# leotimus/binary-recommendation

Hardware: AMD Instinct MI355X
Metric: (user,item) pairs/sec at batch 65536 dim 64 (higher is better)
Workload: dtype f32; 1 GPU; NeuMF-A full training step (trainers/NFC_plain.py graph: 4 embeddings, 128->100->50->10->1, BCE, Keras-Adam adam_dense), embed_dim=64, 1000000 users x 100000 items per GPU, batch 65536 per GPU, uniform ids; global_batch=65536, parallelism=single GPU, steps_per_graph_launch=4, optimizer=adam_dense (deferred replay)

## Files before the change

### binary-recommendation_amd/csrc/dense.h

```cpp
#pragma once
#include "common.h"
#include "philox.h"
#include <stdlib.h>

namespace br {

typedef __bf16 bf16x8 __attribute__((ext_vector_type(8)));
typedef float f32x4_t __attribute__((ext_vector_type(4)));
__device__ __forceinline__ void split3(float x0, float x1, uint32_t& h, uint32_t& m, uint32_t& l) {
  typedef __bf16 bf2 __attribute__((ext_vector_type(2)));
  typedef float f2 __attribute__((ext_vector_type(2)));
  const f2 x = {x0, x1};
  h = __builtin_bit_cast(uint32_t, (bf2){(__bf16)x.x, (__bf16)x.y});
  const f2 hf = {__builtin_bit_cast(float, h << 16), __builtin_bit_cast(float, h & 0xffff0000u)};
  const f2 r = x - hf;
  m = __builtin_bit_cast(uint32_t, (bf2){(__bf16)r.x, (__bf16)r.y});
  const f2 mf = {__builtin_bit_cast(float, m << 16), __builtin_bit_cast(float, m & 0xffff0000u)};
  const f2 t = r - mf;
  l = __builtin_bit_cast(uint32_t, (bf2){(__bf16)t.x, (__bf16)t.y});
}
__device__ __forceinline__ bf16x8 frag8(const uint32_t (&p)[4]) {
  typedef uint32_t u4 __attribute__((ext_vector_type(4)));
  const u4 v = {p[0], p[1], p[2], p[3]};
  return __builtin_bit_cast(bf16x8, v);
}
__device__ __forceinline__ bf16x8 frag8(const float4& q) {
  typedef float f4 __attribute__((ext_vector_type(4)));
  const f4 v = {q.x, q.y, q.z, q.w};
  return __builtin_bit_cast(bf16x8, v);
}
__device__ __forceinline__ f32x4_t mfma_bf16(bf16x8 a, bf16x8 b, f32x4_t c) {
#if defined(__HIP_DEVICE_COMPILE__)
  return __builtin_amdgcn_mfma_f32_16x16x32_bf16(a, b, c, 0, 0, 0);
#else
  return c;
#endif
}
static inline bool mlp_bf16x6() {
  static const bool on = [] { const char* e = getenv("BR_MLP_MATH"); return !(e && e[0] == 'f'); }();
  return on;
}

struct BwdArgs {
  const float* gy; int64_t ldgy;
  const float* y; int64_t ldy;
  const float* x; int64_t ldx;
  const float* W;
  int64_t batch;
  int K, N, act;
  const float* o_mean; const float* o_rstd; const float* o_gamma; const double* o_sums; float inv_batch;
  const float* scale; const float* shift;
  const uint32_t* keep; int kw; float inv_keep;
  const float* i_mean; const float* i_rstd; double* in_sums;
  float* gx; int64_t ldgx;
  float* slabs; int64_t slab_elems; int64_t db_off;
  float* zero = nullptr; int64_t zero_n = 0;
};

int make_keep_args(KeepArgs& a, float drop_p, uint64_t seed, uint32_t step, uint32_t step_add, int64_t row0, int64_t batch, int n_sites,
                   const uint32_t* sites, const int* widths, uint32_t* const* out);
int dropout_keep_bits_ahead(float drop_p, uint64_t seed, uint32_t step, uint32_t step_add, int64_t row0, int64_t batch, int n_sites,
                            const uint32_t* sites, const int* widths, uint32_t* const* out, brStream stream);

struct AdamPairCall {
  float *table_a, *m_a, *v_a; int64_t rows_a; const void* sorted_ids_a; const int32_t* sorted_pos_a; const float* grads_a; int64_t ldg_a;
  const float* grads_hi_a; int64_t ldg_hi_a; uint8_t* mark_a; int32_t* last_a;
  float *table_b, *m_b, *v_b; int64_t rows_b; const void* sorted_ids_b; const int32_t* sorted_pos_b; const float* grads_b; int64_t ldg_b;
  const float* grads_hi_b; int64_t ldg_hi_b; uint8_t* mark_b; int32_t* last_b;
  int dim, id_type; int64_t n; int split; const float* hi_scale; const void* step_state; double alpha_t, beta1, beta2, eps;
  float *seg_ws_a, *seg_ws_b;
  const float *th_lo_a = nullptr, *th_hi_a = nullptr, *th_lo_b = nullptr, *th_hi_b = nullptr; int64_t ld_th = 0;
  const StepAdvance* adv = nullptr;
};
struct FinalArgs;
int adam_rows_pair_keep(const AdamPairCall& c, const KeepArgs* keep, brStream stream, const FinalArgs* fin = nullptr, bool* fin_done = nullptr);

struct LookupArgs;
struct IndexPairArgs {
  void* sorted_ids_a; int32_t* sorted_pos_a; void* ws_a; int64_t ws_a_bytes;
  void* sorted_ids_b; int32_t* sorted_pos_b; void* ws_b; int64_t ws_b_bytes;
};
bool lookup_with_index_supported(int dim, int64_t n, int64_t upper_a, int64_t upper_b, int64_t ld_stash, const void* x0, const void* stash_a, const void* stash_b);
struct GroupIndexArgs { int n = 0; const void* users[BR_GROUP_MAX - 1]; const void* items[BR_GROUP_MAX - 1]; IndexPairArgs ix[BR_GROUP_MAX - 1]; };
int lookup_with_index(const LookupArgs& la, int dim, int id_type, const IndexPairArgs& ix, brStream stream, const StepAdvance* adv = nullptr,
                      const GroupIndexArgs* later = nullptr);
int lookup_index_chunks(int64_t n);
int lookup_wave_launch(const LookupArgs& la, int dim, int id_type, brStream stream);

int dense_backward_fused(const BwdArgs& a, hipStream_t s);
int dense_bwd_fused_grid(int64_t batch);
size_t dense_bwd_fused_lds(int NT, int KT);

struct TailMArgs {
  const float* a2; int64_t lda2;
  const float *W3, *b3, *w4, *b4, *dot, *labels;
  const float *scale2, *shift2, *mean2, *rstd2;
  const double* stats2; double batch_total; const float *gamma2, *beta2; float bn_eps, bn_momentum;
  float *moving_mean, *moving_var, *out_scale, *out_shift, *out_mean, *out_rstd;
  const uint32_t* keep; int kw; float inv_keep;
  int64_t batch;
  int n2, n3, act, mf_first, loss;
  float inv_batch;
  float *a3, *logit, *prob, *ddot, *gh2;
  int64_t ldgh2;
  double *msums, *bn_sums;
  float* slabs; int n_slabs;
};
int tail_mfma_grid(int64_t batch);
void launch_tail_mfma(const TailMArgs& a, int grid, hipStream_t s);

}
```

### binary-recommendation_amd/csrc/stamps.h

```cpp
#pragma once
#include "common.h"

namespace br {

#ifdef BR_STAMPS
constexpr int kStampSlots = 12;
__device__ unsigned long long* g_stamp_buf = nullptr;
#define BR_STAMP_DECL unsigned long long stamps_[kStampSlots] = {0, 0, 0, 0, 0, 0, 0, 0, 0, 0, 0, 0}
#define BR_STAMP(i)                                                                             \
  do {                                                                                          \
    __builtin_amdgcn_sched_barrier(0);                                                          \
    unsigned long long t_;                                                                      \
    asm volatile("s_memtime %0\n\ts_waitcnt lgkmcnt(0)" : "=s"(t_)::"memory");                  \
    if (stamps_[i] == 0) stamps_[i] = t_;                                                       \
    __builtin_amdgcn_sched_barrier(0);                                                          \
  } while (0)
#define BR_STAMP_RT(i)                                                                          \
  do {                                                                                          \
    unsigned long long t_;                                                                      \
    asm volatile("s_memrealtime %0\n\ts_waitcnt lgkmcnt(0)" : "=s"(t_)::"memory");              \
    stamps_[i] = t_;                                                                            \
  } while (0)
#define BR_STAMP_FLUSH(widx)                                                                    \
  do {                                                                                          \
    if ((threadIdx.x & 63) == 0 && g_stamp_buf)                                                 \
      for (int i_ = 0; i_ < kStampSlots; ++i_) g_stamp_buf[(size_t)(widx) * kStampSlots + i_] = stamps_[i_]; \
  } while (0)
#else
#define BR_STAMP_DECL
#define BR_STAMP(i)
#define BR_STAMP_RT(i)
#define BR_STAMP_FLUSH(widx)
#endif

}
```

### binary-recommendation_amd/csrc/tail.hip

```cpp
#include "common.h"
#include "dense.h"

namespace br {

constexpr int kTailRows = 128;
constexpr int kTailLpr = 4;
constexpr int kTailRep = BR_STAT_REPLICAS;

struct TailArgs {
  const float* a2; int64_t lda2;
  const float *W3, *b3, *w4, *b4, *dot, *labels;
  const float *scale2, *shift2, *mean2, *rstd2;
  const uint8_t* keep; int64_t keep_ld; float inv_keep;
  int64_t batch;
  int n2, n3, act, mf_first, loss;
  float inv_batch;
  float *a3, *logit, *prob, *ddot, *gh2;
  int64_t ldgh2;
  double *msums, *bn_sums;
  float* slabs;
};

template <int N3P, int ROWS>
__global__ __launch_bounds__(ROWS * kTailLpr) void neumf_tail_kernel(TailArgs a) {
  constexpr int kTailThreads = ROWS * kTailLpr, kTailWaves = kTailThreads / 64, kPasses = kTailRows / ROWS;
  extern __shared__ __attribute__((aligned(16))) float smem[];
  const int n2 = a.n2, n3 = a.n3, ld = n2 | 1;
  float* A = smem;
  float* X = A + ROWS * ld;
  float* Ws = X + ROWS * ld;
  float* DZ = Ws + n2 * N3P;
  float* cst = DZ + ROWS * (N3P + 1);
  float* hw = cst + 4 * n2;
  float* A3s = hw + 2 * N3P;
  __shared__ float redf[kTailWaves][N3P + 2];
  __shared__ double redd[kTailWaves][BR_METRIC_SUMS];
  __shared__ double colred[2][128];
  const int t = threadIdx.x, lane = t & 63, wave = t >> 6;
  const int r = t >> 2, q = t & 3;
  const int moff = a.mf_first ? 1 : 0;
  const float wdot = a.w4[a.mf_first ? 0 : n3], bias4 = a.b4[0];
  const int64_t base0 = (int64_t)blockIdx.x * kTailRows;
#pragma unroll 1
  for (int pass = 0; pass < kPasses; ++pass) {
  const int64_t base = base0 + (int64_t)pass * ROWS;
  const int64_t left = a.batch - base;
  const int nrow = (int)(left < ROWS ? (left > 0 ? left : 0) : ROWS);
  const bool live = r < nrow;
  const int64_t gr = base + r;
  const float d = live ? a.dot[gr] : 0.f, yv = live ? a.labels[gr] : 0.f;

  {
    constexpr int RPW = ROWS / kTailWaves;
    float v[RPW][2];
#pragma unroll
    for (int i = 0; i < RPW; ++i) {
      const int rr = wave + kTailWaves * i;
      const float* src = a.a2 + (rr < nrow ? base + rr : base0) * a.lda2;
#pragma unroll
      for (int h = 0; h < 2; ++h) {
        const int k = lane + 64 * h;
        const float x = src[k < n2 ? k : 0];
        v[i][h] = (rr < nrow && k < n2) ? x : 0.f;
      }
    }
#pragma unroll
    for (int i = 0; i < RPW; ++i) {
      const int rr = wave + kTailWaves * i;
#pragma unroll
      for (int h = 0; h < 2; ++h) {
        const int k = lane + 64 * h;
        if (k < n2) A[rr * ld + k] = v[i][h];
      }
    }
  }
  if (pass == 0) {
    for (int e = t; e < n2 * N3P; e += kTailThreads) { const int k = e / N3P, n = e - k * N3P; Ws[e] = n < n3 ? a.W3[k * n3 + n] : 0.f; }
    for (int k = t; k < n2; k += kTailThreads) {
      cst[k] = a.scale2[k]; cst[n2 + k] = a.shift2[k]; cst[2 * n2 + k] = a.mean2[k]; cst[3 * n2 + k] = a.rstd2[k];
    }
    for (int n = t; n < N3P; n += kTailThreads) { hw[n] = n < n3 ? a.b3[n] : 0.f; hw[N3P + n] = n < n3 ? a.w4[moff + n] : 0.f; }
  }
  for (int k = t; k < 256; k += kTailThreads) (&colred[0][0])[k] = 0.0;
  __syncthreads();

  const float ik = a.inv_keep;
  float z[N3P];
#pragma unroll
  for (int n = 0; n < N3P; ++n) z[n] = q == 0 ? hw[n] : 0.f;
  uint32_t bits[4];
#pragma unroll
  for (int i = 0; i < 4; ++i) {
    const int k0 = 8 * (q + 4 * i);
    bits[i] = 0u;
    if (k0 < n2) {
      bits[i] = live ? (a.keep ? (uint32_t)a.keep[gr * a.keep_ld + (k0 >> 3)] : 0xFFu) : 0u;
      const int kend = (n2 - k0) < 8 ? (n2 - k0) : 8;
      for (int j = 0; j < kend; ++j) {
        const int k = k0 + j;
        const float h = A[r * ld + k] * cst[k] + cst[n2 + k];
        const float x = ((bits[i] >> j) & 1u) ? h * ik : 0.f;
        X[r * ld + k] = x;
#pragma unroll
        for (int n4 = 0; n4 < N3P; n4 += 4) {
          const float4 w = *reinterpret_cast<const float4*>(Ws + k * N3P + n4);
          z[n4] += x * w.x; z[n4 + 1] += x * w.y; z[n4 + 2] += x * w.z; z[n4 + 3] += x * w.w;
        }
      }
    }
  }
#pragma unroll
  for (int n = 0; n < N3P; ++n) { z[n] += __shfl_xor(z[n], 1, 64); z[n] += __shfl_xor(z[n], 2, 64); }
  float lz = bias4 + d * wdot;
#pragma unroll
  for (int n = 0; n < N3P; ++n) {
    z[n] = n < n3 ? act_apply(z[n], a.act) : 0.f;
    lz += z[n] * hw[N3P + n];
  }
  const float p = sigmoidf_acc(lz);
  float dzl = 0.f;
  double s_loss = 0.0, s_se = 0.0, s_ae = 0.0, s_ok = 0.0, s_bce = 0.0, s_tp = 0.0, s_fp = 0.0, s_fn = 0.0;
  const bool own = live && q == 0;
  if (live) {
    float l;
    const float bce = fmaxf(lz, 0.f) - lz * yv + log1pf(expf(-fabsf(lz)));
    if (a.loss == BR_LOSS_BCE) {
      l = bce;
      dzl = (p - yv) * a.inv_batch;
    } else {
      l = (p - yv) * (p - yv);
      dzl = 2.f * (p - yv) * p * (1.f - p) * a.inv_batch;
    }
    if (own) {
      s_loss = (double)l; s_se = (double)((p - yv) * (p - yv)); s_ae = (double)fabsf(p - yv);
      const bool pp = p > 0.5f, yp = yv > 0.5f;
      s_ok = (pp == yp) ? 1.0 : 0.0;
      s_bce = (double)bce; s_tp = (pp && yp) ? 1.0 : 0.0; s_fp = (pp && !yp) ? 1.0 : 0.0; s_fn = (!pp && yp) ? 1.0 : 0.0;
      a.logit[gr] = lz;
      a.prob[gr] = p;
      a.ddot[gr] = dzl * wdot;
    }
  }
  if (q == 0) {
#pragma unroll
    for (int n = 0; n < N3P; ++n) A3s[r * (N3P + 1) + n] = z[n];
  }
  float dz[N3P];
#pragma unroll
  for (int n = 0; n < N3P; ++n) {
    dz[n] = (live && n < n3) ? dzl * hw[N3P + n] * act_grad_from_out(z[n], a.act) : 0.f;
    if (q == 0) DZ[r * (N3P + 1) + n] = dz[n];
  }
  const float dzo = own ? dzl : 0.f;
#pragma unroll
  for (int n = 0; n < N3P; ++n) {
    const float v = group_sum<64>(dzo * z[n]);
    if (lane == 0) redf[wave][n] = v;
  }
  {
    const float v0 = group_sum<64>(dzo * d), v1 = group_sum<64>(dzo);
    if (lane == 0) { redf[wave][N3P] = v0; redf[wave][N3P + 1] = v1; }
    s_loss = wave_sum_d(s_loss); s_se = wave_sum_d(s_se); s_ae = wave_sum_d(s_ae); s_ok = wave_sum_d(s_ok);
    s_bce = wave_sum_d(s_bce); s_tp = wave_sum_d(s_tp); s_fp = wave_sum_d(s_fp); s_fn = wave_sum_d(s_fn);
    if (lane == 0) {
      redd[wave][0] = s_loss; redd[wave][1] = s_se; redd[wave][2] = s_ae; redd[wave][3] = s_ok;
      redd[wave][4] = s_bce; redd[wave][5] = s_tp; redd[wave][6] = s_fp; redd[wave][7] = s_fn;
    }
  }
  __syncthreads();

  float* slab = a.slabs + (int64_t)blockIdx.x * ((int64_t)n2 * n3 + 2 * n3 + 2);
  for (int o = t; o < n2 * n3; o += kTailThreads) {
    const int k = o / n3, n = o - k * n3;
    float acc = 0.f;
    for (int rr = 0; rr < ROWS; ++rr) acc += X[rr * ld + k] * DZ[rr * (N3P + 1) + n];
    slab[o] = pass ? slab[o] + acc : acc;
  }
  if (a.a3)
    for (int e = t; e < nrow * n3; e += kTailThreads) { const int rr = e / n3; a.a3[base * n3 + e] = A3s[rr * (N3P + 1) + (e - rr * n3)]; }
  auto put = [&](int i, float v) { slab[i] = pass ? slab[i] + v : v; };
  auto wsum = [&](int i) { float v = 0.f; for (int w = 0; w < kTailWaves; ++w) v += redf[w][i]; return v; };
  if (t < n3) {
    float acc = 0.f;
    for (int rr = 0; rr < ROWS; ++rr) acc += DZ[rr * (N3P + 1) + t];
    put(n2 * n3 + t, acc);
    put(n2 * n3 + n3 + moff + t, wsum(t));
  }
  if (t == 64) put(n2 * n3 + n3 + (a.mf_first ? 0 : n3), wsum(N3P));
  if (t == 65) put(n2 * n3 + 2 * n3 + 1, wsum(N3P + 1));
  if (t >= 96 && t < 96 + BR_METRIC_SUMS && a.msums) {
    double v = 0.0;
    for (int w = 0; w < kTailWaves; ++w) v += redd[w][t - 96];
    atomicAdd(a.msums + (size_t)(blockIdx.x & (BR_SUM_SLOTS - 1)) * BR_METRIC_SUMS + (t - 96), v);
  }
  __syncthreads();

#pragma unroll
  for (int i = 0; i < 4; ++i) {
    const int k0 = 8 * (q + 4 * i);
    if (k0 < n2) {
      const int kend = (n2 - k0) < 8 ? (n2 - k0) : 8;
      for (int j = 0; j < kend; ++j) {
        const int k = k0 + j;
        float acc = 0.f;
#pragma unroll
        for (int n4 = 0; n4 < N3P; n4 += 4) {
          const float4 w = *reinterpret_cast<const float4*>(Ws + k * N3P + n4);
          acc += dz[n4] * w.x + dz[n4 + 1] * w.y + dz[n4 + 2] * w.z + dz[n4 + 3] * w.w;
        }
        const float dh = ((bits[i] >> j) & 1u) ? acc * ik : 0.f;
        const float xhat = (A[r * ld + k] - cst[2 * n2 + k]) * cst[3 * n2 + k];
        A[r * ld + k] = dh;
        X[r * ld + k] = dh * xhat;
      }
    }
  }
  __syncthreads();
  if (a.bn_sums) {
    for (int idx = t; idx < 4 * n2; idx += kTailThreads) {
      const int part = idx / n2, k = idx - part * n2;
      float s1 = 0.f, s2 = 0.f;
      for (int rr = part * (ROWS / 4); rr < (part + 1) * (ROWS / 4); ++rr) { s1 += A[rr * ld + k]; s2 += X[rr * ld + k]; }
      atomicAdd(&colred[0][k], (double)s1);
      atomicAdd(&colred[1][k], (double)s2);
    }
  }
  for (int rr = wave; rr < nrow; rr += kTailWaves) {
    float* dst = a.gh2 + (base + rr) * a.ldgh2;
    for (int k = lane; k < n2; k += 64) dst[k] = A[rr * ld + k];
  }
  if (a.bn_sums) {
    __syncthreads();
    double* rep = a.bn_sums + (size_t)(blockIdx.x % kTailRep) * 2 * n2;
    for (int k = t; k < n2; k += kTailThreads) {
      atomicAdd(rep + k, colred[0][k]);
      atomicAdd(rep + n2 + k, colred[1][k]);
    }
  }
  if (kPasses > 1) __syncthreads();
  }
}

static size_t tail_lds_bytes(int n2, int n3p, int rows) {
  const int ld = n2 | 1;
  return sizeof(float) * ((size_t)2 * rows * ld + (size_t)n2 * n3p + (size_t)2 * rows * (n3p + 1) + 4 * (size_t)n2 + 2 * (size_t)n3p);
}
static size_t tail_static_lds_bytes(int n3p, int rows) {
  const int waves = rows * kTailLpr / 64;
  return sizeof(float) * waves * (n3p + 2) + sizeof(double) * (waves * BR_METRIC_SUMS + 2 * 128);
}
constexpr size_t kTailDynLdsMax = 150 * 1024;
constexpr size_t kTailCuLds = 160 * 1024;
static bool tail_fits(int n2, int n3p, int rows) {
  const size_t dyn = tail_lds_bytes(n2, n3p, rows);
  return dyn <= kTailDynLdsMax && dyn + tail_static_lds_bytes(n3p, rows) <= kTailCuLds;
}
static int tail_tile_rows(int n2, int n3p) { return tail_fits(n2, n3p, kTailRows) ? kTailRows : kTailRows / 2; }

}

using namespace br;

extern "C" int brNeumfTailSlabs(int64_t batch) { return (int)ceil_div(batch > 0 ? batch : 1, kTailRows); }

extern "C" int64_t brNeumfTailSlabElems(int n2, int n3) { return (int64_t)n2 * n3 + 2 * n3 + 2; }

extern "C" int brNeumfTailFused(const float* a2, int64_t lda2, const float* W3, const float* b3, const float* w4, const float* b4,
                                const float* dot, const float* labels, const float* scale2, const float* shift2, const float* mean2,
                                const float* rstd2, const brBnFold* bn2, float drop_p, const uint32_t* keep,
                                int64_t batch, int n2, int n3, int act, int mf_first, int loss, float inv_batch, float* a3,
                                float* logit, float* prob, double* sums, float* ddot, float* gh2, int64_t ldgh2, double* bn_sums,
                                float* slabs, int n_slabs, brStream stream) {
  BR_CHECK_ARG(a2 && W3 && b3 && w4 && b4 && dot && labels && logit && prob && ddot && gh2 && slabs, "brNeumfTailFused: null pointer");
  BR_CHECK_ARG(bn2 ? (!scale2 && !shift2 && !mean2 && !rstd2 && bn2->stats && bn2->gamma && bn2->beta && bn2->scale && bn2->shift && bn2->mean && bn2->rstd &&
                      bn2->batch_total > 0 && (bn2->moving_mean == nullptr) == (bn2->moving_var == nullptr))
                   : (scale2 && shift2 && mean2 && rstd2),
               "brNeumfTailFused: BatchNorm 2 either as scale2/shift2/mean2/rstd2 or as bn2 (stats, gamma, beta and the four outputs)");
  BR_CHECK_ARG(batch >= 0 && n2 >= 1 && n2 <= 128 && n3 >= 1 && n3 <= 32 && lda2 >= n2 && ldgh2 >= n2, "brNeumfTailFused: bad sizes");
  BR_CHECK_ARG(drop_p >= 0.f && drop_p < 1.f, "brNeumfTailFused: drop_p out of [0,1)");
  BR_CHECK_ARG((drop_p > 0.f) == (keep != nullptr), "brNeumfTailFused: keep bits (brDropoutKeepBits) are required exactly when drop_p > 0");
  BR_CHECK_ARG(loss == BR_LOSS_BCE || loss == BR_LOSS_MSE, "brNeumfTailFused: bad loss");
  const int n3p = (n3 + 3) & ~3, tile_rows = tail_tile_rows(n2, n3p);
  if (!tail_fits(n2, n3p, tile_rows)) {
    set_error("brNeumfTailFused: n2 = %d with n3 = %d needs %zu B of dynamic LDS (+ %zu B static) for %d-row tiles, above the %zu B a workgroup may "
              "request; the largest supported combination is n2 = 128 with n3 = 32",
              n2, n3, tail_lds_bytes(n2, n3p, tile_rows), tail_static_lds_bytes(n3p, tile_rows), tile_rows, kTailDynLdsMax);
    return BR_ERR_UNSUPPORTED;
  }
  if (batch == 0) return BR_OK;
  BR_CHECK_ARG(n_slabs == brNeumfTailSlabs(batch), "brNeumfTailFused: n_slabs must be brNeumfTailSlabs(batch)");
  hipStream_t s = (hipStream_t)stream;
  const auto al16 = [](const void* p) { return (reinterpret_cast<uintptr_t>(p) & 15) == 0; };
  if (n2 <= 64 && n3 <= 16 && lda2 % 4 == 0 && ldgh2 % 4 == 0 && al16(a2) && al16(gh2)) {
    TailMArgs m{};
    m.a2 = a2; m.lda2 = lda2; m.W3 = W3; m.b3 = b3; m.w4 = w4; m.b4 = b4; m.dot = dot; m.labels = labels;
    m.scale2 = scale2; m.shift2 = shift2; m.mean2 = mean2; m.rstd2 = rstd2;
    if (bn2) {
      m.stats2 = bn2->stats; m.batch_total = bn2->batch_total; m.gamma2 = bn2->gamma; m.beta2 = bn2->beta; m.bn_eps = bn2->eps; m.bn_momentum = bn2->momentum;
      m.moving_mean = bn2->moving_mean; m.moving_var = bn2->moving_var; m.out_scale = bn2->scale; m.out_shift = bn2->shift; m.out_mean = bn2->mean; m.out_rstd = bn2->rstd;
    }
    m.keep = keep; m.kw = (n2 + 31) / 32; m.inv_keep = drop_p > 0.f ? 1.0f / (1.0f - drop_p) : 1.0f;
    m.batch = batch; m.n2 = n2; m.n3 = n3; m.act = act; m.mf_first = mf_first; m.loss = loss; m.inv_batch = inv_batch;
    m.a3 = a3; m.logit = logit; m.prob = prob; m.ddot = ddot; m.gh2 = gh2; m.ldgh2 = ldgh2; m.msums = sums; m.bn_sums = bn_sums; m.slabs = slabs;
    int grid = tail_mfma_grid(batch);
    if (grid > n_slabs) grid = n_slabs;
    m.n_slabs = n_slabs;
    launch_tail_mfma(m, grid, s);
    BR_CHECK_LAUNCH("brNeumfTailFused(mfma)");
    return BR_OK;
  }
  if (bn2) {
    int rc = brBnFinalize(bn2->stats, bn2->batch_total, bn2->gamma, bn2->beta, bn2->eps, bn2->momentum, bn2->moving_mean, bn2->moving_var, bn2->scale,
                          bn2->shift, bn2->mean, bn2->rstd, n2, stream);
    if (rc != BR_OK) return rc;
    scale2 = bn2->scale; shift2 = bn2->shift; mean2 = bn2->mean; rstd2 = bn2->rstd;
  }
  TailArgs a;
  a.a2 = a2; a.lda2 = lda2; a.W3 = W3; a.b3 = b3; a.w4 = w4; a.b4 = b4; a.dot = dot; a.labels = labels;
  a.scale2 = scale2; a.shift2 = shift2; a.mean2 = mean2; a.rstd2 = rstd2;
  a.keep = reinterpret_cast<const uint8_t*>(keep); a.keep_ld = 4 * (int64_t)((n2 + 31) / 32); a.inv_keep = drop_p > 0.f ? 1.0f / (1.0f - drop_p) : 1.0f;
  a.batch = batch; a.n2 = n2; a.n3 = n3; a.act = act; a.mf_first = mf_first; a.loss = loss; a.inv_batch = inv_batch;
  a.a3 = a3; a.logit = logit; a.prob = prob; a.ddot = ddot; a.gh2 = gh2; a.ldgh2 = ldgh2; a.msums = sums; a.bn_sums = bn_sums;
  a.slabs = slabs;
  const size_t lds = tail_lds_bytes(n2, n3p, tile_rows);
  const unsigned grid = (unsigned)n_slabs;
#define BR_TAIL_LAUNCH(NP, ROWS)                                                                                          \
  {                                                                                                                       \
    static bool attr = false;                                                                                             \
    if (!attr) {                                                                                                          \
      const hipError_t e = hipFuncSetAttribute((const void*)neumf_tail_kernel<NP, ROWS>, hipFuncAttributeMaxDynamicSharedMemorySize, (int)kTailDynLdsMax); \
      if (e != hipSuccess) { set_error("brNeumfTailFused: cannot raise the dynamic LDS limit to %zu B: %s", kTailDynLdsMax, hipGetErrorString(e)); return BR_ERR_HIP; } \
      attr = true;                                                                                                        \
    }                                                                                                                     \
    neumf_tail_kernel<NP, ROWS><<<grid, ROWS * kTailLpr, lds, s>>>(a);                                                     \
  }
#define BR_TAIL(NP) case NP: BR_TAIL_LAUNCH(NP, kTailRows) break;
#define BR_TAIL2(NP) case NP: if (tile_rows == kTailRows) BR_TAIL_LAUNCH(NP, kTailRows) else BR_TAIL_LAUNCH(NP, kTailRows / 2) break;
  switch (n3p) {
    BR_TAIL(4) BR_TAIL(8) BR_TAIL2(12) BR_TAIL2(16) BR_TAIL2(20) BR_TAIL2(24) BR_TAIL2(28) BR_TAIL2(32)
    default: set_error("brNeumfTailFused: unsupported n3"); return BR_ERR_UNSUPPORTED;
  }
#undef BR_TAIL
#undef BR_TAIL2
#undef BR_TAIL_LAUNCH
  BR_CHECK_LAUNCH("brNeumfTailFused");
  return BR_OK;
}
```

### binary-recommendation_amd/csrc/tail_mfma.hip

```cpp
#include "dense.h"

namespace br {

using f32x4 = __attribute__((ext_vector_type(4))) float;

constexpr int kTmThreads = 512;
constexpr int kTmWaves = kTmThreads / 64;
constexpr int kTmRep = BR_STAT_REPLICAS;
constexpr int kTmPatchLd = 20;
constexpr int kTmKT = 4;

__device__ __forceinline__ f32x4 mfma16t(float a, float b, f32x4 c) {
  return __builtin_amdgcn_mfma_f32_16x16x4f32(a, b, c, 0, 0, 0);
}
__device__ __forceinline__ float keep_bit_t(float x, uint32_t w, uint32_t pos) {
  return __int_as_float(__float_as_int(x) & __builtin_amdgcn_sbfe((int)w, pos, 1u));
}

struct TailTile {
  float4 av[kTmKT];
  uint32_t ka[2];
  float xr[4][kTmKT], dv[4], yv[4];
  uint32_t kc[4][2];
  int vm[4];
};
__device__ __forceinline__ void tail_load_tile(TailTile& t, const TailMArgs& a, int64_t tile, int c16, int g) {
  const int64_t batch = a.batch, rbase = tile << 4;
  const int n2 = a.n2;
  const int64_t arow = rbase + c16 < batch ? rbase + c16 : batch - 1;
  const float* pa = a.a2 + arow * a.lda2 + 4 * g;
#pragma unroll
  for (int j = 0; j < kTmKT; ++j) t.av[j] = *reinterpret_cast<const float4*>(16 * j + 4 * g < n2 ? pa + 16 * j : pa - 4 * g);
  t.ka[0] = t.ka[1] = 0xFFFFFFFFu;
  if (a.keep) { t.ka[0] = a.keep[arow * a.kw]; t.ka[1] = a.keep[arow * a.kw + (a.kw > 1 ? 1 : 0)]; }
#pragma unroll
  for (int r = 0; r < 4; ++r) {
    const int64_t row = rbase + 4 * g + r;
    t.vm[r] = row < batch ? -1 : 0;
    const int64_t rc = row < batch ? row : batch - 1;
    const float* px = a.a2 + rc * a.lda2;
#pragma unroll
    for (int kt = 0; kt < kTmKT; ++kt) { const int k = kt * 16 + c16; t.xr[r][kt] = px[k < n2 ? k : 0]; }
    t.kc[r][0] = a.keep ? a.keep[rc * a.kw] : 0xFFFFFFFFu;
    t.kc[r][1] = a.keep ? a.keep[rc * a.kw + (a.kw > 1 ? 1 : 0)] : 0xFFFFFFFFu;
    t.dv[r] = a.dot[rc];
    t.yv[r] = a.labels[rc];
  }
}

__global__ __launch_bounds__(kTmThreads, 2) void neumf_tail_mfma_kernel(const TailMArgs a) {
  __shared__ __attribute__((aligned(16))) float Wf[4 * 4 * 16 * 4];
  __shared__ __attribute__((aligned(16))) float Wb[64 * 16];
  __shared__ float cst[4][64];
  __shared__ __attribute__((aligned(16))) float hv[2][16];
  __shared__ __attribute__((aligned(16))) float patches[kTmWaves][16 * kTmPatchLd];
  __shared__ float wsum[kTmWaves][64 * 16];
  __shared__ float wcol[kTmWaves][2][16 + 2];
  __shared__ double wbn[2][64];
  __shared__ double wmet[kTmWaves][BR_METRIC_SUMS];
  const int lane = threadIdx.x & 63, wave = threadIdx.x >> 6;
  const int c16 = lane & 15, g = lane >> 4;
  const int n2 = a.n2, n3 = a.n3;
  const int64_t batch = a.batch;
  const int moff = a.mf_first ? 1 : 0;
  const int sigmask = a.act == BR_ACT_SIGMOID ? -1 : 0, relumask = a.act == BR_ACT_RELU ? -1 : 0;
  const float floor_ = a.act == BR_ACT_RELU ? 0.f : -__builtin_inff();

  const int64_t n_tiles = (batch + 15) >> 4;
  const int64_t tile0 = (int64_t)blockIdx.x * kTmWaves + wave;
  TailTile tt;
  if (tile0 < n_tiles) tail_load_tile(tt, a, tile0, c16, g);
  for (int t = threadIdx.x; t < 64; t += kTmThreads) {
    float sc = 0.f, sh = 0.f, mu = 0.f, rs = 0.f;
    if (t < n2) {
      if (a.stats2) {
        double s1 = 0.0, s2 = 0.0;
        for (int r = 0; r < kTmRep; ++r) { s1 += a.stats2[(size_t)r * 2 * n2 + t]; s2 += a.stats2[(size_t)r * 2 * n2 + n2 + t]; }
        const double m = s1 / a.batch_total;
        double var = s2 / a.batch_total - m * m;
        if (var < 0.0) var = 0.0;
        mu = (float)m;
        const float varf = (float)var;
        rs = 1.0f / sqrtf(varf + a.bn_eps);
        sc = a.gamma2[t] * rs;
        sh = a.beta2[t] - mu * sc;
        if (blockIdx.x == 0) {
          a.out_scale[t] = sc; a.out_shift[t] = sh; a.out_mean[t] = mu; a.out_rstd[t] = rs;
          if (a.moving_mean) {
            a.moving_mean[t] = a.moving_mean[t] * a.bn_momentum + mu * (1.0f - a.bn_momentum);
            a.moving_var[t] = a.moving_var[t] * a.bn_momentum + varf * (1.0f - a.bn_momentum);
          }
        }
      } else { sc = a.scale2[t]; sh = a.shift2[t]; mu = a.mean2[t]; rs = a.rstd2[t]; }
    }
    cst[0][t] = sc; cst[1][t] = sh; cst[2][t] = mu; cst[3][t] = rs;
    wbn[0][t] = 0.0; wbn[1][t] = 0.0;
  }
  for (int t = threadIdx.x; t < 16; t += kTmThreads) {
    hv[0][t] = t < n3 ? a.b3[t] : 0.f;
    hv[1][t] = t < n3 ? a.w4[moff + t] : 0.f;
  }
  for (int t = threadIdx.x; t < 64 * 16; t += kTmThreads) {
    const int k = t >> 4, n = t & 15;
    const float w = (k < n2 && n < n3) ? a.W3[k * n3 + n] : 0.f;
    Wb[t] = w;
    Wf[(((k >> 4) * 4 + ((k >> 2) & 3)) * 16 + n) * 4 + (k & 3)] = w;
  }
  __syncthreads();

  const float wdot = a.w4[a.mf_first ? 0 : n3], bias4 = a.b4[0];
  float* patch = patches[wave];
  f32x4 dW[kTmKT];
#pragma unroll
  for (int kt = 0; kt < kTmKT; ++kt) dW[kt] = (f32x4){0.f, 0.f, 0.f, 0.f};
  float db3 = 0.f, dw4 = 0.f, dw4dot = 0.f, db4 = 0.f;
  float isum[kTmKT], isq[kTmKT];
#pragma unroll
  for (int kt = 0; kt < kTmKT; ++kt) { isum[kt] = 0.f; isq[kt] = 0.f; }
  double s_loss = 0.0, s_se = 0.0, s_ae = 0.0, s_ok = 0.0, s_bce = 0.0, s_tp = 0.0, s_fp = 0.0, s_fn = 0.0;
  const float4 w4q = *reinterpret_cast<const float4*>(&hv[1][4 * g]);
  const float b3c = hv[0][c16], w4c = hv[1][c16];
  const float ik = a.inv_keep;

  for (int64_t tile = tile0; tile < n_tiles; tile += (int64_t)gridDim.x * kTmWaves) {
    const int64_t rbase = tile << 4;
    if (tile != tile0) tail_load_tile(tt, a, tile, c16, g);
    float4 (&av)[kTmKT] = tt.av;
    uint32_t (&ka)[2] = tt.ka;
    float (&xr)[4][kTmKT] = tt.xr;
    float (&dv)[4] = tt.dv;
    float (&yv)[4] = tt.yv;
    uint32_t (&kc)[4][2] = tt.kc;
    int (&vm)[4] = tt.vm;
    f32x4 z = (f32x4){0.f, 0.f, 0.f, 0.f};
#pragma unroll
    for (int j = 0; j < kTmKT; ++j) {
      const int k = 16 * j + 4 * g;
      const float4 sc = *reinterpret_cast<const float4*>(&cst[0][k]), sh = *reinterpret_cast<const float4*>(&cst[1][k]);
      const uint32_t w = ka[j >> 1], p0 = 16u * (j & 1) + 4u * g;
      const float t0 = keep_bit_t(fmaf(av[j].x, sc.x, sh.x), w, p0), t1 = keep_bit_t(fmaf(av[j].y, sc.y, sh.y), w, p0 + 1);
      const float t2 = keep_bit_t(fmaf(av[j].z, sc.z, sh.z), w, p0 + 2), t3 = keep_bit_t(fmaf(av[j].w, sc.w, sh.w), w, p0 + 3);
      const float4 b = *reinterpret_cast<const float4*>(Wf + ((j * 4 + g) * 16 + c16) * 4);
      z = mfma16t(t0, b.x, z); z = mfma16t(t1, b.y, z); z = mfma16t(t2, b.z, z); z = mfma16t(t3, b.w, z);
    }
    const int cm = c16 < n3 ? -1 : 0;
    float a3v[4];
#pragma unroll
    for (int r = 0; r < 4; ++r) {
      const float zz = fmaf(z[r], ik, b3c);
      const float s = __builtin_amdgcn_rcpf(1.0f + __builtin_amdgcn_exp2f(zz * -1.44269504088896340736f));
      const float m = fmaxf(zz, floor_);
      a3v[r] = __int_as_float(((__float_as_int(s) & sigmask) | (__float_as_int(m) & ~sigmask)) & cm);
      patch[(4 * g + r) * kTmPatchLd + c16] = a3v[r];
    }
    __builtin_amdgcn_wave_barrier();
    const float4 ar = *reinterpret_cast<const float4*>(patch + c16 * kTmPatchLd + 4 * g);
    __builtin_amdgcn_wave_barrier();
    f32x4 lzv = (f32x4){0.f, 0.f, 0.f, 0.f};
    lzv = mfma16t(ar.x, w4q.x, lzv); lzv = mfma16t(ar.y, w4q.y, lzv); lzv = mfma16t(ar.z, w4q.z, lzv); lzv = mfma16t(ar.w, w4q.w, lzv);
    float dzl[4];
#pragma unroll
    for (int r = 0; r < 4; ++r) {
      const float lz = lzv[r] + bias4 + dv[r] * wdot;
      const float e = expf(-fabsf(lz));
      const float rinv = 1.0f / (1.0f + e);
      const float p = lz >= 0.f ? rinv : e * rinv;
      float l, d;
      const float bce = fmaxf(lz, 0.f) - lz * yv[r] + log1pf(e);
      if (a.loss == BR_LOSS_BCE) { l = bce; d = (p - yv[r]) * a.inv_batch; }
      else { l = (p - yv[r]) * (p - yv[r]); d = 2.f * (p - yv[r]) * p * (1.f - p) * a.inv_batch; }
      dzl[r] = __int_as_float(__float_as_int(d) & vm[r]);
      if (c16 == 0 && vm[r]) {
        const int64_t row = rbase + 4 * g + r;
        a.logit[row] = lz; a.prob[row] = p; a.ddot[row] = dzl[r] * wdot;
        s_loss += (double)l; s_se += (double)((p - yv[r]) * (p - yv[r])); s_ae += (double)fabsf(p - yv[r]);
        const bool pp = p > 0.5f, yp = yv[r] > 0.5f;
        s_ok += (pp == yp) ? 1.0 : 0.0;
        s_bce += (double)bce; s_tp += (pp && yp) ? 1.0 : 0.0; s_fp += (pp && !yp) ? 1.0 : 0.0; s_fn += (!pp && yp) ? 1.0 : 0.0;
        dw4dot = fmaf(dzl[r], dv[r], dw4dot);
        db4 += dzl[r];
      }
    }
    float dz3[4];
#pragma unroll
    for (int r = 0; r < 4; ++r) {
      const float ds = a3v[r] * (1.f - a3v[r]);
      const float dr = a3v[r] > 0.f ? 1.f : 0.f;
      const float dl = __int_as_float((__float_as_int(ds) & sigmask) | (__float_as_int(dr) & relumask) | (0x3f800000 & ~(sigmask | relumask)));
      dz3[r] = __int_as_float(__float_as_int(dzl[r] * w4c * dl) & cm);
      dw4 = fmaf(dzl[r], a3v[r], dw4);
      db3 += dz3[r];
      patch[(4 * g + r) * kTmPatchLd + c16] = dz3[r];
      if (a.a3 && c16 < n3 && vm[r]) a.a3[(rbase + 4 * g + r) * n3 + c16] = a3v[r];
    }
    __builtin_amdgcn_wave_barrier();
    const float4 dzr = *reinterpret_cast<const float4*>(patch + c16 * kTmPatchLd + 4 * g);
    __builtin_amdgcn_wave_barrier();
    const bool row_ok = rbase + c16 < batch;
    float* ghrow = a.gh2 + (rbase + (row_ok ? c16 : 0)) * a.ldgh2 + 4 * g;
#pragma unroll
    for (int kt = 0; kt < kTmKT; ++kt) {
      const int k = kt * 16 + c16;
      const float4 b = *reinterpret_cast<const float4*>(Wb + k * 16 + 4 * g);
      f32x4 gh = (f32x4){0.f, 0.f, 0.f, 0.f};
      gh = mfma16t(dzr.x, b.x, gh); gh = mfma16t(dzr.y, b.y, gh); gh = mfma16t(dzr.z, b.z, gh); gh = mfma16t(dzr.w, b.w, gh);
      const float sck = cst[0][k], shk = cst[1][k], muk = cst[2][k], rsk = cst[3][k];
#pragma unroll
      for (int r = 0; r < 4; ++r) {
        const uint32_t w = kc[r][kt >> 1], pos = 16u * (kt & 1) + c16;
        const float dh = keep_bit_t(gh[r] * ik, w, pos);
        isum[kt] += dh;
        isq[kt] = fmaf(dh, (xr[r][kt] - muk) * rsk, isq[kt]);
        patch[(4 * g + r) * kTmPatchLd + c16] = dh;
        const float tx = keep_bit_t(fmaf(xr[r][kt], sck, shk), w, pos);
        dW[kt] = mfma16t(tx, dz3[r], dW[kt]);
      }
      __builtin_amdgcn_wave_barrier();
      const float4 o = *reinterpret_cast<const float4*>(patch + c16 * kTmPatchLd + 4 * g);
      __builtin_amdgcn_wave_barrier();
      if (row_ok && kt * 16 + 4 * g < n2) *reinterpret_cast<float4*>(ghrow + kt * 16) = o;
    }
  }

#pragma unroll
  for (int kt = 0; kt < kTmKT; ++kt) {
#pragma unroll
    for (int r = 0; r < 4; ++r) wsum[wave][(kt * 16 + 4 * g + r) * 16 + c16] = dW[kt][r];
    float sv = isum[kt], q = isq[kt];
    sv += __shfl_xor(sv, 16, 64); sv += __shfl_xor(sv, 32, 64);
    q += __shfl_xor(q, 16, 64); q += __shfl_xor(q, 32, 64);
    if (g == 0) { atomicAdd(&wbn[0][kt * 16 + c16], (double)sv); atomicAdd(&wbn[1][kt * 16 + c16], (double)q); }
  }
  {
    float v0 = db3, v1 = dw4;
    v0 += __shfl_xor(v0, 16, 64); v0 += __shfl_xor(v0, 32, 64);
    v1 += __shfl_xor(v1, 16, 64); v1 += __shfl_xor(v1, 32, 64);
    if (g == 0) { wcol[wave][0][c16] = v0; wcol[wave][1][c16] = v1; }
    float u0 = c16 == 0 ? dw4dot : 0.f, u1 = c16 == 0 ? db4 : 0.f;
    u0 = group_sum<64>(u0); u1 = group_sum<64>(u1);
    if (lane == 0) { wcol[wave][0][16] = u0; wcol[wave][0][17] = u1; }
    s_loss = wave_sum_d(s_loss); s_se = wave_sum_d(s_se); s_ae = wave_sum_d(s_ae); s_ok = wave_sum_d(s_ok);
    s_bce = wave_sum_d(s_bce); s_tp = wave_sum_d(s_tp); s_fp = wave_sum_d(s_fp); s_fn = wave_sum_d(s_fn);
    if (lane == 0) {
      wmet[wave][0] = s_loss; wmet[wave][1] = s_se; wmet[wave][2] = s_ae; wmet[wave][3] = s_ok;
      wmet[wave][4] = s_bce; wmet[wave][5] = s_tp; wmet[wave][6] = s_fp; wmet[wave][7] = s_fn;
    }
  }
  __syncthreads();
  const int64_t slab_el = (int64_t)n2 * n3 + 2 * n3 + 2;
  float* slab = a.slabs + (int64_t)blockIdx.x * slab_el;
  for (int64_t sl = (int64_t)blockIdx.x + gridDim.x; sl < a.n_slabs; sl += gridDim.x)
    for (int t = threadIdx.x; t < slab_el; t += kTmThreads) a.slabs[sl * slab_el + t] = 0.f;
  for (int t = threadIdx.x; t < 64 * 16; t += kTmThreads) {
    const int k = t >> 4, n = t & 15;
    if (k < n2 && n < n3) {
      float s = 0.f;
#pragma unroll
      for (int w = 0; w < kTmWaves; ++w) s += wsum[w][t];
      slab[k * n3 + n] = s * ik;
    }
  }
  if (threadIdx.x < 18) {
    const int t = threadIdx.x;
    float s0 = 0.f, s1 = 0.f;
#pragma unroll
    for (int w = 0; w < kTmWaves; ++w) { s0 += wcol[w][0][t]; s1 += t < 16 ? wcol[w][1][t] : 0.f; }
    if (t < n3) { slab[n2 * n3 + t] = s0; slab[n2 * n3 + n3 + moff + t] = s1; }
    if (t == 16) slab[n2 * n3 + n3 + (a.mf_first ? 0 : n3)] = s0;
    if (t == 17) slab[n2 * n3 + 2 * n3 + 1] = s0;
  }
  if (threadIdx.x >= 64 && threadIdx.x < 64 + BR_METRIC_SUMS && a.msums) {
    const int t = threadIdx.x - 64;
    double v = 0.0;
#pragma unroll
    for (int w = 0; w < kTmWaves; ++w) v += wmet[w][t];
    atomicAdd(a.msums + (size_t)(blockIdx.x & (BR_SUM_SLOTS - 1)) * BR_METRIC_SUMS + t, v);
  }
  if (a.bn_sums && threadIdx.x >= 128 && threadIdx.x < 128 + 64) {
    const int k = threadIdx.x - 128;
    if (k < n2) {
      double* rep = a.bn_sums + (size_t)(blockIdx.x % kTmRep) * 2 * n2;
      atomicAdd(rep + k, wbn[0][k]);
      atomicAdd(rep + n2 + k, wbn[1][k]);
    }
  }
}

int tail_mfma_grid(int64_t batch) {
  const int64_t t = ceil_div(ceil_div(batch > 0 ? batch : 1, 16), kTmWaves);
  return (int)(t < 1 ? 1 : (t > 256 ? 256 : t));
}
void launch_tail_mfma(const TailMArgs& a, int grid, hipStream_t s) { neumf_tail_mfma_kernel<<<(unsigned)grid, kTmThreads, 0, s>>>(a); }

}
```

Before: 230.9 million pairs/s.

## Add slim tail-tile form with next-tile prefetch and batched wave reductions

Adds a templated 'slim' form of the NeuMF tail MFMA kernel, on by default. Each wave loads a compact tile (row-major activations plus keep bits, dot and label), prefetches the next tile while working on the current one, and uses an LDS patch to get the transposed x values instead of loading them from global memory. It also batches the end-of-kernel shuffle reductions, hoists the W3/b3/w4 loads ahead of the BN-stat reduction, and adds timestamp probes that compile only under BR_STAMPS. The costs are more LDS per block, which may lower occupancy, and a second register set for the prefetched tile.

```diff
diff --git a/binary-recommendation_amd/csrc/dense.h b/binary-recommendation_amd/csrc/dense.h
--- a/binary-recommendation_amd/csrc/dense.h
+++ b/binary-recommendation_amd/csrc/dense.h
@@ -107,6 +107,6 @@
   float* slabs; int n_slabs;
 };
 int tail_mfma_grid(int64_t batch);
-void launch_tail_mfma(const TailMArgs& a, int grid, hipStream_t s);
+void launch_tail_mfma(const TailMArgs& a, int grid, int form, hipStream_t s);
 
 }
diff --git a/binary-recommendation_amd/csrc/stamps.h b/binary-recommendation_amd/csrc/stamps.h
--- a/binary-recommendation_amd/csrc/stamps.h
+++ b/binary-recommendation_amd/csrc/stamps.h
@@ -15,6 +15,11 @@
     if (stamps_[i] == 0) stamps_[i] = t_;                                                       \
     __builtin_amdgcn_sched_barrier(0);                                                          \
   } while (0)
+#define BR_STAMP_LANDED(i)                                                                      \
+  do {                                                                                          \
+    asm volatile("s_waitcnt vmcnt(0)" ::: "memory");                                            \
+    BR_STAMP(i);                                                                                \
+  } while (0)
 #define BR_STAMP_RT(i)                                                                          \
   do {                                                                                          \
     unsigned long long t_;                                                                      \
@@ -29,6 +34,7 @@
 #else
 #define BR_STAMP_DECL
 #define BR_STAMP(i)
+#define BR_STAMP_LANDED(i)
 #define BR_STAMP_RT(i)
 #define BR_STAMP_FLUSH(widx)
 #endif
diff --git a/binary-recommendation_amd/csrc/tail.hip b/binary-recommendation_amd/csrc/tail.hip
--- a/binary-recommendation_amd/csrc/tail.hip
+++ b/binary-recommendation_amd/csrc/tail.hip
@@ -305,7 +305,8 @@
     int grid = tail_mfma_grid(batch);
     if (grid > n_slabs) grid = n_slabs;
     m.n_slabs = n_slabs;
-    launch_tail_mfma(m, grid, s);
+    const char* e = getenv("BR_TAIL_FORM");
+    launch_tail_mfma(m, grid, (e && e[0] == '0') ? 0 : 1, s);
     BR_CHECK_LAUNCH("brNeumfTailFused(mfma)");
     return BR_OK;
   }
diff --git a/binary-recommendation_amd/csrc/tail_mfma.hip b/binary-recommendation_amd/csrc/tail_mfma.hip
--- a/binary-recommendation_amd/csrc/tail_mfma.hip
+++ b/binary-recommendation_amd/csrc/tail_mfma.hip
@@ -1,4 +1,5 @@
 #include "dense.h"
+#include "stamps.h"
 
 namespace br {
 
@@ -9,6 +10,7 @@
 constexpr int kTmRep = BR_STAT_REPLICAS;
 constexpr int kTmPatchLd = 20;
 constexpr int kTmKT = 4;
+constexpr int kTmXLd = 68;
 
 __device__ __forceinline__ f32x4 mfma16t(float a, float b, f32x4 c) {
   return __builtin_amdgcn_mfma_f32_16x16x4f32(a, b, c, 0, 0, 0);
@@ -48,7 +50,27 @@
   }
 }
 
+struct TailTileSlim {
+  float4 av[kTmKT];
+  uint32_t ka[2];
+  float dv, yv;
+};
+__device__ __forceinline__ void tail_load_slim(TailTileSlim& t, const TailMArgs& a, int64_t tile, int c16, int g) {
+  const int64_t batch = a.batch, rbase = tile << 4;
+  const int n2 = a.n2;
+  const int64_t arow = rbase + c16 < batch ? rbase + c16 : batch - 1;
+  const float* pa = a.a2 + arow * a.lda2 + 4 * g;
+#pragma unroll
+  for (int j = 0; j < kTmKT; ++j) t.av[j] = *reinterpret_cast<const float4*>(16 * j + 4 * g < n2 ? pa + 16 * j : pa - 4 * g);
+  t.ka[0] = t.ka[1] = 0xFFFFFFFFu;
+  if (a.keep) { t.ka[0] = a.keep[arow * a.kw]; t.ka[1] = a.keep[arow * a.kw + (a.kw > 1 ? 1 : 0)]; }
+  t.dv = a.dot[arow];
+  t.yv = a.labels[arow];
+}
+
+template <int FORM>
 __global__ __launch_bounds__(kTmThreads, 2) void neumf_tail_mfma_kernel(const TailMArgs a) {
+  constexpr bool kSlim = FORM != 0;
   __shared__ __attribute__((aligned(16))) float Wf[4 * 4 * 16 * 4];
   __shared__ __attribute__((aligned(16))) float Wb[64 * 16];
   __shared__ float cst[4][64];
@@ -62,20 +84,45 @@
   const int c16 = lane & 15, g = lane >> 4;
   const int n2 = a.n2, n3 = a.n3;
   const int64_t batch = a.batch;
+  BR_STAMP_DECL;
+  BR_STAMP_RT(10);
+  BR_STAMP(0);
+  float* xpatch = nullptr;
+  if constexpr (kSlim) {
+    __shared__ __attribute__((aligned(16))) float xpatches[kTmWaves][16 * kTmXLd];
+    xpatch = xpatches[wave];
+  }
   const int moff = a.mf_first ? 1 : 0;
   const int sigmask = a.act == BR_ACT_SIGMOID ? -1 : 0, relumask = a.act == BR_ACT_RELU ? -1 : 0;
   const float floor_ = a.act == BR_ACT_RELU ? 0.f : -__builtin_inff();
 
   const int64_t n_tiles = (batch + 15) >> 4;
-  const int64_t tile0 = (int64_t)blockIdx.x * kTmWaves + wave;
+  const int64_t tile0 = (int64_t)blockIdx.x * kTmWaves + wave, tile_step = (int64_t)gridDim.x * kTmWaves;
   TailTile tt;
-  if (tile0 < n_tiles) tail_load_tile(tt, a, tile0, c16, g);
+  TailTileSlim cur;
+  if (tile0 < n_tiles) {
+    if constexpr (kSlim) tail_load_slim(cur, a, tile0, c16, g);
+    else tail_load_tile(tt, a, tile0, c16, g);
+  }
+  BR_STAMP(1);
+  static_assert(64 * 16 == 2 * kTmThreads, "two W3 image elements per thread");
+  float w3v[2], hvv[2] = {0.f, 0.f};
+#pragma unroll
+  for (int i = 0; i < 2; ++i) {
+    const int t = threadIdx.x + i * kTmThreads, k = t >> 4, n = t & 15;
+    w3v[i] = (k < n2 && n < n3) ? a.W3[k * n3 + n] : 0.f;
+  }
+  if (threadIdx.x < 16 && (int)threadIdx.x < n3) { hvv[0] = a.b3[threadIdx.x]; hvv[1] = a.w4[moff + threadIdx.x]; }
   for (int t = threadIdx.x; t < 64; t += kTmThreads) {
     float sc = 0.f, sh = 0.f, mu = 0.f, rs = 0.f;
     if (t < n2) {
       if (a.stats2) {
+        double v1[kTmRep], v2[kTmRep];
+#pragma unroll
+        for (int r = 0; r < kTmRep; ++r) { v1[r] = a.stats2[(size_t)r * 2 * n2 + t]; v2[r] = a.stats2[(size_t)r * 2 * n2 + n2 + t]; }
         double s1 = 0.0, s2 = 0.0;
-        for (int r = 0; r < kTmRep; ++r) { s1 += a.stats2[(size_t)r * 2 * n2 + t]; s2 += a.stats2[(size_t)r * 2 * n2 + n2 + t]; }
+#pragma unroll
+        for (int r = 0; r < kTmRep; ++r) { s1 += v1[r]; s2 += v2[r]; }
         const double m = s1 / a.batch_total;
         double var = s2 / a.batch_total - m * m;
         if (var < 0.0) var = 0.0;
@@ -96,19 +143,18 @@
     cst[0][t] = sc; cst[1][t] = sh; cst[2][t] = mu; cst[3][t] = rs;
     wbn[0][t] = 0.0; wbn[1][t] = 0.0;
   }
-  for (int t = threadIdx.x; t < 16; t += kTmThreads) {
-    hv[0][t] = t < n3 ? a.b3[t] : 0.f;
-    hv[1][t] = t < n3 ? a.w4[moff + t] : 0.f;
-  }
-  for (int t = threadIdx.x; t < 64 * 16; t += kTmThreads) {
-    const int k = t >> 4, n = t & 15;
-    const float w = (k < n2 && n < n3) ? a.W3[k * n3 + n] : 0.f;
-    Wb[t] = w;
-    Wf[(((k >> 4) * 4 + ((k >> 2) & 3)) * 16 + n) * 4 + (k & 3)] = w;
+  if (threadIdx.x < 16) { hv[0][threadIdx.x] = hvv[0]; hv[1][threadIdx.x] = hvv[1]; }
+#pragma unroll
+  for (int i = 0; i < 2; ++i) {
+    const int t = threadIdx.x + i * kTmThreads, k = t >> 4, n = t & 15;
+    Wb[t] = w3v[i];
+    Wf[(((k >> 4) * 4 + ((k >> 2) & 3)) * 16 + n) * 4 + (k & 3)] = w3v[i];
   }
   __syncthreads();
-
-  const float wdot = a.w4[a.mf_first ? 0 : n3], bias4 = a.b4[0];
+  BR_STAMP(2);
+
+  const float wdot = __int_as_float(__builtin_amdgcn_readfirstlane(__float_as_int(a.w4[a.mf_first ? 0 : n3])));
+  const float bias4 = __int_as_float(__builtin_amdgcn_readfirstlane(__float_as_int(a.b4[0])));
   float* patch = patches[wave];
   f32x4 dW[kTmKT];
 #pragma unroll
@@ -122,16 +168,38 @@
   const float b3c = hv[0][c16], w4c = hv[1][c16];
   const float ik = a.inv_keep;
 
-  for (int64_t tile = tile0; tile < n_tiles; tile += (int64_t)gridDim.x * kTmWaves) {
+  for (int64_t tile = tile0; tile < n_tiles; tile += tile_step) {
     const int64_t rbase = tile << 4;
-    if (tile != tile0) tail_load_tile(tt, a, tile, c16, g);
-    float4 (&av)[kTmKT] = tt.av;
-    uint32_t (&ka)[2] = tt.ka;
-    float (&xr)[4][kTmKT] = tt.xr;
-    float (&dv)[4] = tt.dv;
-    float (&yv)[4] = tt.yv;
-    uint32_t (&kc)[4][2] = tt.kc;
-    int (&vm)[4] = tt.vm;
+    float4 av[kTmKT];
+    uint32_t ka[2], kc[4][2];
+    float dv[4], yv[4];
+    int vm[4];
+    TailTileSlim nxt{};
+    if constexpr (kSlim) {
+      if (tile + tile_step < n_tiles) tail_load_slim(nxt, a, tile + tile_step, c16, g);
+      if (tile != tile0) { BR_STAMP_LANDED(6); }
+      ka[0] = cur.ka[0]; ka[1] = cur.ka[1];
+#pragma unroll
+      for (int j = 0; j < kTmKT; ++j) {
+        av[j] = cur.av[j];
+        *reinterpret_cast<float4*>(xpatch + c16 * kTmXLd + 16 * j + 4 * g) = av[j];
+      }
+#pragma unroll
+      for (int r = 0; r < 4; ++r) {
+        const int src = 4 * g + r;
+        kc[r][0] = __shfl(ka[0], src, 64); kc[r][1] = __shfl(ka[1], src, 64);
+        dv[r] = __shfl(cur.dv, src, 64); yv[r] = __shfl(cur.yv, src, 64);
+        vm[r] = rbase + src < batch ? -1 : 0;
+      }
+      __builtin_amdgcn_wave_barrier();
+    } else {
+      if (tile != tile0) { tail_load_tile(tt, a, tile, c16, g); BR_STAMP_LANDED(6); }
+      ka[0] = tt.ka[0]; ka[1] = tt.ka[1];
+#pragma unroll
+      for (int j = 0; j < kTmKT; ++j) av[j] = tt.av[j];
+#pragma unroll
+      for (int r = 0; r < 4; ++r) { kc[r][0] = tt.kc[r][0]; kc[r][1] = tt.kc[r][1]; dv[r] = tt.dv[r]; yv[r] = tt.yv[r]; vm[r] = tt.vm[r]; }
+    }
     f32x4 z = (f32x4){0.f, 0.f, 0.f, 0.f};
 #pragma unroll
     for (int j = 0; j < kTmKT; ++j) {
@@ -143,6 +211,7 @@
       const float4 b = *reinterpret_cast<const float4*>(Wf + ((j * 4 + g) * 16 + c16) * 4);
       z = mfma16t(t0, b.x, z); z = mfma16t(t1, b.y, z); z = mfma16t(t2, b.z, z); z = mfma16t(t3, b.w, z);
     }
+    BR_STAMP(3);
     const int cm = c16 < n3 ? -1 : 0;
     float a3v[4];
 #pragma unroll
@@ -181,6 +250,7 @@
         db4 += dzl[r];
       }
     }
+    BR_STAMP(4);
     float dz3[4];
 #pragma unroll
     for (int r = 0; r < 4; ++r) {
@@ -205,14 +275,20 @@
       f32x4 gh = (f32x4){0.f, 0.f, 0.f, 0.f};
       gh = mfma16t(dzr.x, b.x, gh); gh = mfma16t(dzr.y, b.y, gh); gh = mfma16t(dzr.z, b.z, gh); gh = mfma16t(dzr.w, b.w, gh);
       const float sck = cst[0][k], shk = cst[1][k], muk = cst[2][k], rsk = cst[3][k];
+      float xr[4];
+#pragma unroll
+      for (int r = 0; r < 4; ++r) {
+        if constexpr (kSlim) xr[r] = xpatch[(4 * g + r) * kTmXLd + k];
+        else xr[r] = tt.xr[r][kt];
+      }
 #pragma unroll
       for (int r = 0; r < 4; ++r) {
         const uint32_t w = kc[r][kt >> 1], pos = 16u * (kt & 1) + c16;
         const float dh = keep_bit_t(gh[r] * ik, w, pos);
         isum[kt] += dh;
-        isq[kt] = fmaf(dh, (xr[r][kt] - muk) * rsk, isq[kt]);
+        isq[kt] = fmaf(dh, (xr[r] - muk) * rsk, isq[kt]);
         patch[(4 * g + r) * kTmPatchLd + c16] = dh;
-        const float tx = keep_bit_t(fmaf(xr[r][kt], sck, shk), w, pos);
+        const float tx = keep_bit_t(fmaf(xr[r], sck, shk), w, pos);
         dW[kt] = mfma16t(tx, dz3[r], dW[kt]);
       }
       __builtin_amdgcn_wave_barrier();
@@ -220,32 +296,53 @@
       __builtin_amdgcn_wave_barrier();
       if (row_ok && kt * 16 + 4 * g < n2) *reinterpret_cast<float4*>(ghrow + kt * 16) = o;
     }
+    if (tile == tile0) { BR_STAMP(5); } else { BR_STAMP(7); }
+    if constexpr (kSlim) cur = nxt;
   }
 
 #pragma unroll
   for (int kt = 0; kt < kTmKT; ++kt) {
 #pragma unroll
     for (int r = 0; r < 4; ++r) wsum[wave][(kt * 16 + 4 * g + r) * 16 + c16] = dW[kt][r];
-    float sv = isum[kt], q = isq[kt];
-    sv += __shfl_xor(sv, 16, 64); sv += __shfl_xor(sv, 32, 64);
-    q += __shfl_xor(q, 16, 64); q += __shfl_xor(q, 32, 64);
-    if (g == 0) { atomicAdd(&wbn[0][kt * 16 + c16], (double)sv); atomicAdd(&wbn[1][kt * 16 + c16], (double)q); }
   }
   {
-    float v0 = db3, v1 = dw4;
-    v0 += __shfl_xor(v0, 16, 64); v0 += __shfl_xor(v0, 32, 64);
-    v1 += __shfl_xor(v1, 16, 64); v1 += __shfl_xor(v1, 32, 64);
-    if (g == 0) { wcol[wave][0][c16] = v0; wcol[wave][1][c16] = v1; }
-    float u0 = c16 == 0 ? dw4dot : 0.f, u1 = c16 == 0 ? db4 : 0.f;
-    u0 = group_sum<64>(u0); u1 = group_sum<64>(u1);
-    if (lane == 0) { wcol[wave][0][16] = u0; wcol[wave][0][17] = u1; }
-    s_loss = wave_sum_d(s_loss); s_se = wave_sum_d(s_se); s_ae = wave_sum_d(s_ae); s_ok = wave_sum_d(s_ok);
-    s_bce = wave_sum_d(s_bce); s_tp = wave_sum_d(s_tp); s_fp = wave_sum_d(s_fp); s_fn = wave_sum_d(s_fn);
+    constexpr int kCs = 2 * kTmKT + 2;
+    float cs[kCs], ct[kCs];
+#pragma unroll
+    for (int kt = 0; kt < kTmKT; ++kt) { cs[kt] = isum[kt]; cs[kTmKT + kt] = isq[kt]; }
+    cs[2 * kTmKT] = db3; cs[2 * kTmKT + 1] = dw4;
+#pragma unroll
+    for (int off = 16; off <= 32; off <<= 1) {
+#pragma unroll
+      for (int i = 0; i < kCs; ++i) ct[i] = __shfl_xor(cs[i], off, 64);
+#pragma unroll
+      for (int i = 0; i < kCs; ++i) cs[i] += ct[i];
+    }
+    if (g == 0) {
+#pragma unroll
+      for (int kt = 0; kt < kTmKT; ++kt) { atomicAdd(&wbn[0][kt * 16 + c16], (double)cs[kt]); atomicAdd(&wbn[1][kt * 16 + c16], (double)cs[kTmKT + kt]); }
+      wcol[wave][0][c16] = cs[2 * kTmKT]; wcol[wave][1][c16] = cs[2 * kTmKT + 1];
+    }
+    float us[2] = {c16 == 0 ? dw4dot : 0.f, c16 == 0 ? db4 : 0.f}, ut[2];
+    double ms[BR_METRIC_SUMS] = {s_loss, s_se, s_ae, s_ok, s_bce, s_tp, s_fp, s_fn}, mt[BR_METRIC_SUMS];
+#pragma unroll
+    for (int off = 32; off >= 16; off >>= 1) {
+#pragma unroll
+      for (int i = 0; i < 2; ++i) ut[i] = __shfl_xor(us[i], off, 64);
+#pragma unroll
+      for (int i = 0; i < BR_METRIC_SUMS; ++i) mt[i] = __shfl_xor(ms[i], off, 64);
+#pragma unroll
+      for (int i = 0; i < 2; ++i) us[i] += ut[i];
+#pragma unroll
+      for (int i = 0; i < BR_METRIC_SUMS; ++i) ms[i] += mt[i];
+    }
     if (lane == 0) {
-      wmet[wave][0] = s_loss; wmet[wave][1] = s_se; wmet[wave][2] = s_ae; wmet[wave][3] = s_ok;
-      wmet[wave][4] = s_bce; wmet[wave][5] = s_tp; wmet[wave][6] = s_fp; wmet[wave][7] = s_fn;
-    }
-  }
+      wcol[wave][0][16] = us[0]; wcol[wave][0][17] = us[1];
+#pragma unroll
+      for (int i = 0; i < BR_METRIC_SUMS; ++i) wmet[wave][i] = ms[i];
+    }
+  }
+  BR_STAMP(9);
   __syncthreads();
   const int64_t slab_el = (int64_t)n2 * n3 + 2 * n3 + 2;
   float* slab = a.slabs + (int64_t)blockIdx.x * slab_el;
@@ -284,12 +381,18 @@
       atomicAdd(rep + n2 + k, wbn[1][k]);
     }
   }
+  BR_STAMP(8);
+  BR_STAMP_RT(11);
+  BR_STAMP_FLUSH(blockIdx.x * kTmWaves + wave);
 }
 
 int tail_mfma_grid(int64_t batch) {
   const int64_t t = ceil_div(ceil_div(batch > 0 ? batch : 1, 16), kTmWaves);
   return (int)(t < 1 ? 1 : (t > 256 ? 256 : t));
 }
-void launch_tail_mfma(const TailMArgs& a, int grid, hipStream_t s) { neumf_tail_mfma_kernel<<<(unsigned)grid, kTmThreads, 0, s>>>(a); }
-
-}
+void launch_tail_mfma(const TailMArgs& a, int grid, int form, hipStream_t s) {
+  if (form == 0) neumf_tail_mfma_kernel<0><<<(unsigned)grid, kTmThreads, 0, s>>>(a);
+  else neumf_tail_mfma_kernel<1><<<(unsigned)grid, kTmThreads, 0, s>>>(a);
+}
+
+}
```

After: 232.7 million pairs/s (median of 6 runs). About the same (+0.8%).
